# dusk-network/schnorr

Measured on NVIDIA B200. Metric: verifies_per_s, higher is better.
Workload: dtype u32

## Files before the change

### schnorr_b200/csrc/hades.cuh

```cuda
#pragma once
#include "fq.cuh"

namespace sb200 {

#define SB_HADES_W 5

struct HadesTables {
  uint32_t rc[335][8];
  uint32_t mds[25][8];
  uint32_t pre[5][8];
  uint32_t sparse[59 * 11][8];
  uint32_t post[25][8];
};
#if defined(__CUDACC__)
__constant__ HadesTables d_hades;
#endif
static HadesTables h_hades;

#if defined(__CUDA_ARCH__)
#define SB_CONST(name) d_##name
#define SB_HADES(field) d_hades.field
#else
#define SB_CONST(name) h_##name
#define SB_HADES(field) h_hades.field
#endif

SB_HD fq ld8(const uint32_t* p) {
  fq r;
#pragma unroll
  for (int i = 0; i < 8; i++) r.v[i] = p[i];
  return r;
}

SB_HD fq fq_pow5(const fq& x) {
  fq x2 = fq_sqr(x);
  fq x4 = fq_sqr(x2);
  return fq_mul(x4, x);
}

#define SB_MATMUL5(s, mat)                                                                  \
  do {                                                                                      \
    fq _r[5];                                                                               \
    _Pragma("unroll") for (int _k = 0; _k < 5; _k++)                                        \
        _r[_k] = fq_dot5(&SB_HADES(mat)[_k * 5], s[0], s[1], s[2], s[3], s[4]);             \
    _Pragma("unroll") for (int _k = 0; _k < 5; _k++) s[_k] = _r[_k];                        \
  } while (0)

#define SB_MATMUL5_PLAIN(s, mat)                                        \
  do {                                                                  \
    fq _r[5];                                                           \
    _Pragma("unroll 1") for (int _k = 0; _k < 5; _k++) {                \
      fq _a = fq_mul(ld8(SB_HADES(mat)[_k * 5]), s[0]);                 \
      _Pragma("unroll") for (int _j = 1; _j < 5; _j++)                  \
          _a = fq_add(_a, fq_mul(ld8(SB_HADES(mat)[_k * 5 + _j]), s[_j])); \
      _r[_k] = _a;                                                      \
    }                                                                   \
    _Pragma("unroll") for (int _k = 0; _k < 5; _k++) s[_k] = _r[_k];    \
  } while (0)

template <bool LAZY = true>
SB_HD void hades_full_round(fq* s, int rc_base) {
#pragma unroll
  for (int k = 0; k < 5; k++) s[k] = fq_pow5(fq_add(s[k], ld8(SB_HADES(rc)[rc_base + k])));
  if (LAZY) SB_MATMUL5(s, mds); else SB_MATMUL5_PLAIN(s, mds);
}

SB_HD void hades_perm_dense(fq* s) {
  int rc = 0;
#pragma unroll 1
  for (int r = 0; r < 4; r++, rc += 5) hades_full_round<false>(s, rc);
#pragma unroll 1
  for (int r = 0; r < 59; r++, rc += 5) {
#pragma unroll
    for (int k = 0; k < 5; k++) s[k] = fq_add(s[k], ld8(SB_HADES(rc)[rc + k]));
    s[4] = fq_pow5(s[4]);
    SB_MATMUL5_PLAIN(s, mds);
  }
#pragma unroll 1
  for (int r = 0; r < 4; r++, rc += 5) hades_full_round<false>(s, rc);
}

SB_HD void hades_perm(fq* s) {
  int rc = 0;
#pragma unroll 1
  for (int r = 0; r < 4; r++, rc += 5) hades_full_round(s, rc);
#pragma unroll
  for (int k = 0; k < 4; k++) s[k] = fq_add(s[k], ld8(SB_HADES(pre)[k]));
#pragma unroll 1
  for (int t = 0; t < 59; t++) {
    const uint32_t(*c)[8] = &SB_HADES(sparse)[t * 11];
    s[4] = fq_pow5(fq_add(s[4], ld8(c[0])));
    fq np = fq_dot5(&c[1], s[0], s[1], s[2], s[3], s[4]);
#pragma unroll
    for (int j = 0; j < 4; j++) s[j] = fq_add(s[j], fq_mul(ld8(c[6 + j]), s[4]));
    s[4] = np;
  }
  SB_MATMUL5(s, post);
  rc += 59 * 5;
#pragma unroll 1
  for (int r = 0; r < 4; r++, rc += 5) hades_full_round(s, rc);
}

SB_HD void truncate250(const fq& mont_word, uint32_t* c) {
  fq x = fq_from_mont(mont_word);
#pragma unroll
  for (int i = 0; i < 8; i++) c[i] = x.v[i];
  c[7] &= 0x03ffffffu;
}

template <bool DENSE = false>
SB_HD void challenge3(const fq& Ru, const fq& Rv, const fq& m, uint32_t* c) {
  fq s[5] = {fq_zero(), Ru, Rv, m, fq_one()};
  if (DENSE) hades_perm_dense(s); else hades_perm(s);
  truncate250(s[1], c);
}

template <bool DENSE = false>
SB_HD void challenge5(const fq& Ru, const fq& Rv, const fq& Rpu, const fq& Rpv, const fq& m, uint32_t* c) {
  fq s[5] = {fq_zero(), Ru, Rv, Rpu, Rpv};
  if (DENSE) hades_perm_dense(s); else hades_perm(s);
  s[1] = fq_add(s[1], m);
  s[2] = fq_add(s[2], fq_one());
  if (DENSE) hades_perm_dense(s); else hades_perm(s);
  truncate250(s[1], c);
}

}
```

### schnorr_b200/csrc/params_host.cuh

```cuda
#pragma once
#include <cstring>

#include "wire.cuh"

namespace sb200 {
namespace params {

struct Sha512 {
  static uint64_t rotr(uint64_t x, int n) { return (x >> n) | (x << (64 - n)); }
  static void digest(const uint8_t* msg, size_t len, uint8_t out[64]) {
    static const uint64_t K[80] = {
        0x428a2f98d728ae22ull, 0x7137449123ef65cdull, 0xb5c0fbcfec4d3b2full, 0xe9b5dba58189dbbcull, 0x3956c25bf348b538ull,
        0x59f111f1b605d019ull, 0x923f82a4af194f9bull, 0xab1c5ed5da6d8118ull, 0xd807aa98a3030242ull, 0x12835b0145706fbeull,
        0x243185be4ee4b28cull, 0x550c7dc3d5ffb4e2ull, 0x72be5d74f27b896full, 0x80deb1fe3b1696b1ull, 0x9bdc06a725c71235ull,
        0xc19bf174cf692694ull, 0xe49b69c19ef14ad2ull, 0xefbe4786384f25e3ull, 0x0fc19dc68b8cd5b5ull, 0x240ca1cc77ac9c65ull,
        0x2de92c6f592b0275ull, 0x4a7484aa6ea6e483ull, 0x5cb0a9dcbd41fbd4ull, 0x76f988da831153b5ull, 0x983e5152ee66dfabull,
        0xa831c66d2db43210ull, 0xb00327c898fb213full, 0xbf597fc7beef0ee4ull, 0xc6e00bf33da88fc2ull, 0xd5a79147930aa725ull,
        0x06ca6351e003826full, 0x142929670a0e6e70ull, 0x27b70a8546d22ffcull, 0x2e1b21385c26c926ull, 0x4d2c6dfc5ac42aedull,
        0x53380d139d95b3dfull, 0x650a73548baf63deull, 0x766a0abb3c77b2a8ull, 0x81c2c92e47edaee6ull, 0x92722c851482353bull,
        0xa2bfe8a14cf10364ull, 0xa81a664bbc423001ull, 0xc24b8b70d0f89791ull, 0xc76c51a30654be30ull, 0xd192e819d6ef5218ull,
        0xd69906245565a910ull, 0xf40e35855771202aull, 0x106aa07032bbd1b8ull, 0x19a4c116b8d2d0c8ull, 0x1e376c085141ab53ull,
        0x2748774cdf8eeb99ull, 0x34b0bcb5e19b48a8ull, 0x391c0cb3c5c95a63ull, 0x4ed8aa4ae3418acbull, 0x5b9cca4f7763e373ull,
        0x682e6ff3d6b2b8a3ull, 0x748f82ee5defb2fcull, 0x78a5636f43172f60ull, 0x84c87814a1f0ab72ull, 0x8cc702081a6439ecull,
        0x90befffa23631e28ull, 0xa4506cebde82bde9ull, 0xbef9a3f7b2c67915ull, 0xc67178f2e372532bull, 0xca273eceea26619cull,
        0xd186b8c721c0c207ull, 0xeada7dd6cde0eb1eull, 0xf57d4f7fee6ed178ull, 0x06f067aa72176fbaull, 0x0a637dc5a2c898a6ull,
        0x113f9804bef90daeull, 0x1b710b35131c471bull, 0x28db77f523047d84ull, 0x32caab7b40c72493ull, 0x3c9ebe0a15c9bebcull,
        0x431d67c49c100d4cull, 0x4cc5d4becb3e42b6ull, 0x597f299cfc657e2aull, 0x5fcb6fab3ad6faecull, 0x6c44198c4a475817ull};
    uint64_t h[8] = {0x6a09e667f3bcc908ull, 0xbb67ae8584caa73bull, 0x3c6ef372fe94f82bull, 0xa54ff53a5f1d36f1ull,
                     0x510e527fade682d1ull, 0x9b05688c2b3e6c1full, 0x1f83d9abfb41bd6bull, 0x5be0cd19137e2179ull};
    uint8_t buf[256];
    size_t total = ((len + 17 + 127) / 128) * 128;
    if (total > sizeof(buf)) return;
    memset(buf, 0, total);
    memcpy(buf, msg, len);
    buf[len] = 0x80;
    uint64_t bits = (uint64_t)len * 8;
    for (int i = 0; i < 8; i++) buf[total - 1 - i] = (uint8_t)(bits >> (8 * i));
    for (size_t off = 0; off < total; off += 128) {
      uint64_t w[80];
      for (int i = 0; i < 16; i++) {
        uint64_t x = 0;
        for (int k = 0; k < 8; k++) x = (x << 8) | buf[off + 8 * i + k];
        w[i] = x;
      }
      for (int i = 16; i < 80; i++) {
        uint64_t s0 = rotr(w[i - 15], 1) ^ rotr(w[i - 15], 8) ^ (w[i - 15] >> 7);
        uint64_t s1 = rotr(w[i - 2], 19) ^ rotr(w[i - 2], 61) ^ (w[i - 2] >> 6);
        w[i] = w[i - 16] + s0 + w[i - 7] + s1;
      }
      uint64_t a = h[0], b = h[1], c = h[2], d = h[3], e = h[4], f = h[5], g = h[6], hh = h[7];
      for (int i = 0; i < 80; i++) {
        uint64_t S1 = rotr(e, 14) ^ rotr(e, 18) ^ rotr(e, 41), ch = (e & f) ^ (~e & g);
        uint64_t t1 = hh + S1 + ch + K[i] + w[i];
        uint64_t S0 = rotr(a, 28) ^ rotr(a, 34) ^ rotr(a, 39), mj = (a & b) ^ (a & c) ^ (b & c);
        uint64_t t2 = S0 + mj;
        hh = g; g = f; f = e; e = d + t1; d = c; c = b; b = a; a = t1 + t2;
      }
      h[0] += a; h[1] += b; h[2] += c; h[3] += d; h[4] += e; h[5] += f; h[6] += g; h[7] += hh;
    }
    for (int i = 0; i < 8; i++)
      for (int k = 0; k < 8; k++) out[8 * i + k] = (uint8_t)(h[i] >> (56 - 8 * k));
  }
};

inline fq ld(const uint32_t* p) { fq r; memcpy(r.v, p, 32); return r; }
inline void st(uint32_t* p, const fq& a) { memcpy(p, a.v, 32); }
inline fq fq_small(uint32_t x) {
  fq c = fq_zero();
  c.v[0] = x;
  return fq_to_mont(c);
}

inline void default_round_constants(int rule, uint32_t (*out)[8], int n) {
  uint8_t bytes[64];
  const char* seed = "poseidon-for-plonk";
  size_t len = strlen(seed);
  memcpy(bytes, seed, len);
  fq p = fq_one();
  for (int i = 0; i < n; i++) {
    uint8_t d[64];
    Sha512::digest(bytes, len, d);
    memcpy(bytes, d, 64);
    len = 64;
    uint32_t w[16];
    memcpy(w, d, 64);
    fq h = fq_from_wide(w);
    if (rule == SB200_ARK_CUMSUM) {
      h = fq_add(h, p);
      p = h;
    }
    st(out[i], h);
  }
}

inline void default_mds(uint32_t (*out)[5][8]) {
  for (int i = 0; i < 5; i++)
    for (int j = 0; j < 5; j++) st(out[i][j], fq_inv(fq_small((uint32_t)(i + j + 5))));
}

struct Mat4 {
  fq a[4][4];
};
inline Mat4 mat_ident() {
  Mat4 m;
  for (int i = 0; i < 4; i++)
    for (int j = 0; j < 4; j++) m.a[i][j] = i == j ? fq_one() : fq_zero();
  return m;
}
inline Mat4 mat_mul(const Mat4& x, const Mat4& y) {
  Mat4 r;
  for (int i = 0; i < 4; i++)
    for (int j = 0; j < 4; j++) {
      fq s = fq_zero();
      for (int k = 0; k < 4; k++) s = fq_add(s, fq_mul(x.a[i][k], y.a[k][j]));
      r.a[i][j] = s;
    }
  return r;
}
inline void mat_vec(const Mat4& m, const fq* v, fq* out) {
  for (int i = 0; i < 4; i++) {
    fq s = fq_zero();
    for (int k = 0; k < 4; k++) s = fq_add(s, fq_mul(m.a[i][k], v[k]));
    out[i] = s;
  }
}
inline bool mat_inv(const Mat4& m, Mat4& out) {
  fq w[4][8];
  for (int i = 0; i < 4; i++)
    for (int j = 0; j < 8; j++) w[i][j] = j < 4 ? m.a[i][j] : (j - 4 == i ? fq_one() : fq_zero());
  for (int c = 0; c < 4; c++) {
    int piv = -1;
    for (int r = c; r < 4 && piv < 0; r++)
      if (!fq_is_zero(w[r][c])) piv = r;
    if (piv < 0) return false;
    if (piv != c)
      for (int j = 0; j < 8; j++) { fq t = w[c][j]; w[c][j] = w[piv][j]; w[piv][j] = t; }
    fq iv = fq_inv(w[c][c]);
    for (int j = 0; j < 8; j++) w[c][j] = fq_mul(w[c][j], iv);
    for (int r = 0; r < 4; r++) {
      if (r == c || fq_is_zero(w[r][c])) continue;
      fq f = w[r][c];
      for (int j = 0; j < 8; j++) w[r][j] = fq_sub(w[r][j], fq_mul(f, w[c][j]));
    }
  }
  for (int i = 0; i < 4; i++)
    for (int j = 0; j < 4; j++) out.a[i][j] = w[i][4 + j];
  return true;
}

inline bool derive_hades_tables(const uint32_t (*rc)[8], const uint32_t (*mds)[5][8], HadesTables& T) {
  constexpr int W = 5, P = 4, NP = 59, NF = 4;
  memcpy(T.rc, rc, sizeof(T.rc));
  memcpy(T.mds, mds, sizeof(T.mds));
  Mat4 Moo;
  fq Mop[4], Mpo[4], Mpp = ld(mds[P][P]);
  for (int i = 0; i < 4; i++) {
    for (int j = 0; j < 4; j++) Moo.a[i][j] = ld(mds[i][j]);
    Mop[i] = ld(mds[i][P]);
    Mpo[i] = ld(mds[P][i]);
  }
  static thread_local fq folds[NP][4], rows[NP][4], cols[NP][4], F[NP + 1][4];
  Mat4 B = mat_ident();
  for (int t = 0; t < NP; t++) {
    const uint32_t(*c)[8] = rc + (NF + t) * W;
    Mat4 Binv, Bn, Bninv;
    if (!mat_inv(B, Binv)) return false;
    fq co[4];
    for (int i = 0; i < 4; i++) co[i] = ld(c[i]);
    mat_vec(Binv, co, folds[t]);
    Bn = mat_mul(Moo, B);
    if (!mat_inv(Bn, Bninv)) return false;
    mat_vec(Bninv, Mop, cols[t]);
    for (int j = 0; j < 4; j++) {
      fq s = fq_zero();
      for (int k = 0; k < 4; k++) s = fq_add(s, fq_mul(Mpo[k], B.a[k][j]));
      rows[t][j] = s;
    }
    B = Bn;
  }
  for (int k = 0; k < 4; k++) F[0][k] = fq_zero();
  for (int t = 0; t < NP; t++)
    for (int k = 0; k < 4; k++) F[t + 1][k] = fq_add(F[t][k], folds[t][k]);
  for (int k = 0; k < 4; k++) st(T.pre[k], F[NP][k]);
  st(T.pre[P], fq_zero());
  for (int t = 0; t < NP; t++) {
    fq kP = ld(rc[(NF + t) * W + P]);
    if (t > 0) {
      fq corr = fq_zero();
      for (int k = 0; k < 4; k++) corr = fq_add(corr, fq_mul(rows[t - 1][k], fq_sub(F[NP][k], F[t][k])));
      kP = fq_sub(kP, corr);
    }
    uint32_t(*o)[8] = &T.sparse[t * 11];
    st(o[0], kP);
    for (int j = 0; j < 4; j++) st(o[1 + j], rows[t][j]);
    st(o[1 + P], Mpp);
    for (int j = 0; j < 4; j++) st(o[6 + j], cols[t][j]);
    st(o[6 + P], fq_zero());
  }
  for (int i = 0; i < W; i++)
    for (int j = 0; j < W; j++) {
      fq v = (i < 4 && j < 4) ? B.a[i][j] : (i == P && j == P ? fq_one() : fq_zero());
      st(T.post[i * W + j], v);
    }
  return true;
}

inline bool on_curve(const fq& u, const fq& v) {
  fq u2 = fq_sqr(u), v2 = fq_sqr(v);
  return fq_eq(fq_sub(v2, u2), fq_add(fq_one(), fq_mul(ed_d(), fq_mul(u2, v2))));
}
inline bool prime_order(const fq& u, const fq& v) {
  const uint32_t rr[8] = SB200_FR_MOD_INIT;
  ext base = affine_to_ext(u, v), acc = ext_identity();
  pniels nb = ext_to_pniels(base);
  for (int bit = 251; bit >= 0; bit--) {
    acc = p1p1_to_ext(ed_dbl(acc.X, acc.Y, acc.Z));
    if ((rr[bit >> 5] >> (bit & 31)) & 1u) acc = p1p1_to_ext(ed_add(acc, nb));
  }
  const bool is_id = fq_is_zero(acc.X) && fq_eq(acc.Y, acc.Z);
  const bool base_id = fq_is_zero(u) && fq_eq(v, fq_one());
  return is_id && !base_id;
}
inline bool canonical_fq(const uint32_t* p) { return lt_q(p); }

}
}
```

### schnorr_b200/csrc/schnorr_b200.cu

```cuda
#include <cuda_runtime.h>

#include <algorithm>
#include <atomic>
#include <cstdio>
#include <cstring>
#include <mutex>
#include <string>
#include <vector>

#include <map>
#include <thread>

#include "../../include/schnorr_b200.h"
#include "wire.cuh"
#include "params_host.cuh"

using namespace sb200;

namespace {

#ifndef SB_EC_GLOBAL_TABLES
#define SB_EC_GLOBAL_TABLES 1
#endif
constexpr int TPB = 128;
// ... 1075 lines not shown
    };
    for (int k = 0; k < d.nout; k++)
      if (d.out[k]) a.out[k] = dout[k] = (uint32_t*)carve(p, out_bytes(k));
    if (scr) {
      a.scratch = carve(p, scr);
      if (splits_with_scratch(d)) a.out[0] = (uint32_t*)a.scratch;
    }
    uint32_t* dbm = nullptr;
    if (d.bitmap) a.bitmap = dbm = (uint32_t*)carve(p, bm_bytes);
    if ((rc = launch(ctx, d.op, a, st))) return rc;
    auto d2h = [&](uint32_t* host_dst, const uint32_t* dev_src, size_t bytes, bool pinned) -> int {
      uint8_t* dst = (uint8_t*)host_dst;
      if (!pinned) {
        uint8_t* sp = carve(ho_p, bytes);
        dc.pending[slot].push_back({dst, sp, bytes});
        dst = sp;
      }
      CU(cudaMemcpyAsync(dst, dev_src, bytes, cudaMemcpyDeviceToHost, st));
      return SB200_OK;
    };
    for (int k = 0; k < d.nout; k++)
      if (d.out[k] && (rc = d2h(d.out_words[k] < 0 ? d.out[k] + c0 / 32 : d.out[k] + (size_t)c0 * d.out_words[k], dout[k],
                                out_bytes(k), d.out_words[k] < 0 ? bm_pinned : out_pinned[k])))
        return rc;
    if (d.bitmap && (rc = d2h(d.bitmap + c0 / 32, dbm, bm_bytes, bm_pinned))) return rc;
    CU(cudaEventRecord(dc.done[slot], st));
  }
  for (int s = 0; s < 2; s++) {
    int rc = drain_slot(ctx, dc, s);
    if (rc) return rc;
    CU(cudaStreamSynchronize(dc.stream[s]));
  }
  return SB200_OK;
}

void quiesce(DevCtx& dc) {
  cudaSetDevice(dc.dev);
  for (int s = 0; s < 2; s++) {
    if (dc.stream[s]) cudaStreamSynchronize(dc.stream[s]);
    dc.pending[s].clear();
  }
  cudaGetLastError();
}

int run(sb200_ctx* ctx, int64_t n, const Desc& d) {
  if (!ctx || n < 0) return SB200_ERR_ARG;
  uint32_t allowed = SB200_POINTS_AFFINE | SB200_DEVICE_PTRS;
  if (d.op == OP_VERIFY && SB_VERIFY_WS) allowed |= SB200_VERIFY_DUAL_PIPE;
  if (d.op == OP_VERIFY || d.op == OP_VERIFY_DOUBLE || d.op == OP_VERIFY_VARGEN) allowed |= SB200_CHECK_POINTS;
  if (d.op == OP_SIGN || d.op == OP_SIGN_DOUBLE || d.op == OP_SIGN_VARGEN || d.op == OP_KEYGEN || d.op == OP_KEYGEN_DOUBLE ||
      d.op == OP_KEYGEN_VARGEN)
    allowed |= SB200_SIGN_OBLIVIOUS;
  if (d.flags & ~allowed) return SB200_ERR_ARG;
  for (int k = 0; k < d.nin; k++)
    if (d.in_words[k] && (!d.in[k] || ((uintptr_t)d.in[k] & 15))) return SB200_ERR_ARG;
  for (int k = 0; k < d.nout; k++)
    if (d.out[k] && ((uintptr_t)d.out[k] & 15)) return SB200_ERR_ARG;
  if (n == 0) return SB200_OK;
  std::lock_guard<std::mutex> lock(ctx->mu);
  ctx->set_err("");
  DeviceGuard guard;

  if (d.flags & SB200_DEVICE_PTRS) {
    if (ctx->devs.size() != 1) return SB200_ERR_ARG;
    DevCtx& dc = ctx->devs[0];
    CU(cudaSetDevice(dc.dev));
    cudaStream_t st = ctx->user_stream;
    if (dc.user_ev_valid && dc.last_user_stream != st) CU(cudaStreamWaitEvent(st, dc.user_ev, 0));
    KArgs a{};
    a.n = n; a.flags = d.flags; a.aux = d.aux; a.combG = dc.combG; a.combGp = dc.combGp; a.bitmap = d.bitmap;
    a.comb4G = dc.comb4; a.comb4Gp = dc.comb4 + CT_TABLE_WORDS;
    a.ws = dc.ws[2]; a.nsm = dc.nsm; a.ec_scratch = dc.ec_scratch[2]; a.persist = ctx->persist;
    for (int k = 0; k < d.nin; k++) a.in[k] = d.in[k];
    for (int k = 0; k < d.nout; k++) a.out[k] = d.out[k];
    if (const size_t need = scratch_bytes(d, n)) {
      if (dc.cscratch_cap < need) {
        if (dc.user_ev_valid) CU(cudaEventSynchronize(dc.user_ev));
        if (dc.cscratch) CU(cudaFree(dc.cscratch));
        dc.cscratch = nullptr; dc.cscratch_cap = 0;
        if (cudaMalloc(&dc.cscratch, need) != cudaSuccess) { ctx->set_err("cudaMalloc scratch"); return SB200_ERR_NOMEM; }
        dc.cscratch_cap = need;
      }
      a.scratch = (uint8_t*)dc.cscratch;
      if (splits_with_scratch(d)) a.out[0] = dc.cscratch;
    }
    int rc = launch(ctx, d.op, a, st);
    if (rc) return rc;
    CU(cudaEventRecord(dc.user_ev, st));
    dc.user_ev_valid = true;
    dc.last_user_stream = st;
    return SB200_OK;
  }

  size_t per_tuple = 0;
  bool in_pinned[MAX_IN] = {}, out_pinned[MAX_OUT] = {}, bm_pinned = true;
  for (int k = 0; k < d.nin; k++) {
    per_tuple += (size_t)d.in_words[k] * 4;
    if (d.in_words[k]) in_pinned[k] = host_pinned(d.in[k]);
  }
  for (int k = 0; k < d.nout; k++) {
    per_tuple += (d.out[k] && d.out_words[k] > 0) ? (size_t)d.out_words[k] * 4 : 0;
    if (d.out[k]) out_pinned[k] = host_pinned(d.out[k]);
    if (d.out[k] && d.out_words[k] < 0) bm_pinned = bm_pinned && out_pinned[k];
  }
  if (d.bitmap) bm_pinned = bm_pinned && host_pinned(d.bitmap);

  const int ndev = (int)ctx->devs.size();
  const int64_t per_dev = ((n + ndev - 1) / ndev + 31) & ~(int64_t)31;
  std::vector<int> rcs(ndev, SB200_OK);
  auto work = [&](int di) {
    const int64_t lo = std::min<int64_t>(n, di * per_dev), hi = std::min<int64_t>(n, lo + per_dev);
    if (lo < hi) rcs[di] = run_device(ctx, ctx->devs[di], d, lo, hi, per_tuple, in_pinned, out_pinned, bm_pinned);
  };
  if (ndev == 1) {
    work(0);
  } else {
    std::vector<std::thread> th;
    for (int di = 1; di < ndev; di++) th.emplace_back(work, di);
    work(0);
    for (auto& t : th) t.join();
  }
  int rc = SB200_OK;
  for (int di = 0; di < ndev; di++)
    if (rcs[di] && !rc) rc = rcs[di];
  if (rc)
    for (auto& dc : ctx->devs) quiesce(dc);
  return rc;
}

int pt_words(uint32_t flags) { return (flags & SB200_POINTS_AFFINE) ? 16 : 24; }

void release_device(DevCtx& dc) {
  cudaSetDevice(dc.dev);
  for (int s = 0; s < 2; s++) {
    if (dc.stream[s]) { cudaStreamSynchronize(dc.stream[s]); cudaStreamDestroy(dc.stream[s]); }
    if (dc.done[s]) cudaEventDestroy(dc.done[s]);
    if (dc.arena[s]) cudaFree(dc.arena[s]);
    if (dc.hin[s].p) cudaFreeHost(dc.hin[s].p);
    if (dc.hout[s].p) cudaFreeHost(dc.hout[s].p);
  }
  if (dc.user_ev) { if (dc.user_ev_valid) cudaEventSynchronize(dc.user_ev); cudaEventDestroy(dc.user_ev); }
  if (dc.combG) cudaFree(dc.combG);
  if (dc.combGp) cudaFree(dc.combGp);
  if (dc.comb4) cudaFree(dc.comb4);
  for (int s = 0; s < 3; s++) {
    if (dc.ws[s]) cudaFree(dc.ws[s]);
    if (dc.ec_scratch[s]) cudaFree(dc.ec_scratch[s]);
  }
  if (dc.cscratch) cudaFree(dc.cscratch);
  if (dc.registered) {
    std::lock_guard<std::mutex> l(g_params_mu);
    auto it = g_dev_params.find(dc.dev);
    if (it != g_dev_params.end() && --it->second.refs <= 0) g_dev_params.erase(it);
  }
  dc = DevCtx();
}

int prepare_params(const sb200_params* p, HadesTables& T) {
  if (!p || p->struct_size != sizeof(sb200_params) || p->reserved != 0) return SB200_ERR_ARG;
  const uint32_t* all = p->generator;
  const size_t nfe = (sizeof(sb200_params) - 8) / 32;
  for (size_t i = 0; i < nfe; i++)
    if (!params::canonical_fq(all + 8 * i)) return SB200_ERR_PARAMS;
  const fq gu = params::ld(p->generator), gv = params::ld(p->generator + 8);
  const fq hu = params::ld(p->generator_nums), hv = params::ld(p->generator_nums + 8);
  if (!params::on_curve(gu, gv) || !params::on_curve(hu, hv)) return SB200_ERR_PARAMS;
  if (!params::prime_order(gu, gv) || !params::prime_order(hu, hv)) return SB200_ERR_PARAMS;
  if (!params::derive_hades_tables(p->round_constants, p->mds, T)) return SB200_ERR_PARAMS;
  h_hades = T;
  uint64_t s = 0x9e3779b97f4a7c15ull;
  for (int trial = 0; trial < 3; trial++) {
    fq a[5], b[5];
    for (int k = 0; k < 5; k++) {
      for (int j = 0; j < 8; j++) { s ^= s << 13; s ^= s >> 7; s ^= s << 17; a[k].v[j] = trial ? (uint32_t)s : 0u; }
      a[k].v[7] &= 0x3fffffffu;
      b[k] = a[k];
    }
    hades_perm_dense(a);
    hades_perm(b);
    for (int k = 0; k < 5; k++)
      if (!fq_eq(a[k], b[k])) return SB200_ERR_PARAMS;
  }
  return SB200_OK;
}

}

extern "C" {

int sb200_default_params(int ark_rule, sb200_params* out) {
  if (!out) return SB200_ERR_ARG;
  if (ark_rule == SB200_ARK_ENV) {
    const char* e = getenv("SB200_ARK");
    ark_rule = (e && !strcmp(e, "plain")) ? SB200_ARK_PLAIN : SB200_ARK_CUMSUM;
    if (e && strcmp(e, "plain") && strcmp(e, "cumsum") && *e) return SB200_ERR_ARG;
  }
  if (ark_rule != SB200_ARK_CUMSUM && ark_rule != SB200_ARK_PLAIN) return SB200_ERR_ARG;
  memset(out, 0, sizeof(*out));
  out->struct_size = sizeof(sb200_params);
  const uint32_t g[4][8] = {SB200_G_U_INIT, SB200_G_V_INIT, SB200_GP_U_INIT, SB200_GP_V_INIT};
  memcpy(out->generator, g[0], 32); memcpy(out->generator + 8, g[1], 32);
  memcpy(out->generator_nums, g[2], 32); memcpy(out->generator_nums + 8, g[3], 32);
  params::default_round_constants(ark_rule, out->round_constants, 335);
  params::default_mds(out->mds);
  return SB200_OK;
}

int sb200_init(const int* devices, int n_devices, sb200_ctx** out) {
  sb200_params p;
  int rc = sb200_default_params(SB200_ARK_ENV, &p);
  if (rc) return rc;
  return sb200_init_ex(&p, devices, n_devices, out);
}

int sb200_init_ex(const sb200_params* params_in, const int* devices, int n_devices, sb200_ctx** out) {
  if (!out || n_devices < 0 || (n_devices > 0 && !devices)) return SB200_ERR_ARG;
  *out = nullptr;
  sb200_ctx* ctx = new sb200_ctx();
  auto fail = [&](int code) { sb200_destroy(ctx); return code; };
  int rc = prepare_params(params_in, ctx->tables);
  if (rc) return fail(rc);
  ctx->params = *params_in;
  if (const char* e = getenv("SB200_CURVE_PERSISTENT")) ctx->persist = !strcmp(e, "always") ? 1 : !strcmp(e, "never") ? 2 : 0;
  int count = 0;
  if (cudaGetDeviceCount(&count) != cudaSuccess || count == 0) return fail(SB200_ERR_NODEV);
  DeviceGuard guard;
  int dflt = 0;
  if (n_devices == 0) { devices = &dflt; n_devices = 1; }
  const uint64_t hash = fnv1a(params_in, sizeof(*params_in));
  const fq gu = params::ld(params_in->generator), gv = params::ld(params_in->generator + 8);
  const fq hu = params::ld(params_in->generator_nums), hv = params::ld(params_in->generator_nums + 8);
  ctx->devs.reserve(n_devices);
  for (int i = 0; i < n_devices; i++) {
    if (devices[i] < 0 || devices[i] >= count) return fail(SB200_ERR_ARG);
    cudaDeviceProp prop;
    if (cudaGetDeviceProperties(&prop, devices[i]) != cudaSuccess || prop.major < 10) return fail(SB200_ERR_NODEV);
    ctx->devs.emplace_back();
    DevCtx& dc = ctx->devs.back();
    dc.dev = devices[i];
    if (cudaSetDevice(dc.dev) != cudaSuccess) return fail(SB200_ERR_CUDA);
    {
      std::lock_guard<std::mutex> l(g_params_mu);
      DevParams& dp = g_dev_params[dc.dev];
      if (dp.refs > 0 && dp.hash != hash) return fail(SB200_ERR_BUSY);
      if (dp.refs == 0 || dp.hash != hash) {
        if (cudaMemcpyToSymbol(d_hades, &ctx->tables, sizeof(HadesTables)) != cudaSuccess) return fail(SB200_ERR_CUDA);
        dp.hash = hash;
      }
      dp.refs++;
      dc.registered = true;
    }
    for (int s = 0; s < 2; s++) {
      if (cudaStreamCreateWithFlags(&dc.stream[s], cudaStreamNonBlocking) != cudaSuccess) return fail(SB200_ERR_CUDA);
      if (cudaEventCreateWithFlags(&dc.done[s], cudaEventDisableTiming) != cudaSuccess) return fail(SB200_ERR_CUDA);
    }
    if (cudaEventCreateWithFlags(&dc.user_ev, cudaEventDisableTiming) != cudaSuccess) return fail(SB200_ERR_CUDA);
    size_t tb = (size_t)COMB_WINDOWS * COMB_ENTRIES * 24 * 4;
    if (cudaMalloc(&dc.combG, tb) != cudaSuccess || cudaMalloc(&dc.combGp, tb) != cudaSuccess) return fail(SB200_ERR_NOMEM);
    if (cudaMalloc(&dc.comb4, (size_t)2 * CT_TABLE_WORDS * 4) != cudaSuccess) return fail(SB200_ERR_NOMEM);
    if (cudaFuncSetAttribute(k_fixed_batch<OP_SIGN_DOUBLE, true>, cudaFuncAttributeMaxDynamicSharedMemorySize, 2 * CT_TABLE_WORDS * 4) != cudaSuccess ||
        cudaFuncSetAttribute(k_fixed_batch<OP_KEYGEN_DOUBLE, true>, cudaFuncAttributeMaxDynamicSharedMemorySize, 2 * CT_TABLE_WORDS * 4) != cudaSuccess ||
        cudaFuncSetAttribute(k_fixed_batch<OP_SIGN, true>, cudaFuncAttributeMaxDynamicSharedMemorySize, CT_TABLE_WORDS * 4) != cudaSuccess ||
        cudaFuncSetAttribute(k_fixed_batch<OP_KEYGEN, true>, cudaFuncAttributeMaxDynamicSharedMemorySize, CT_TABLE_WORDS * 4) != cudaSuccess)
      return fail(SB200_ERR_CUDA);
    dc.nsm = prop.multiProcessorCount;
#if SB_VERIFY_WS
    if (cudaFuncSetAttribute(k_verify_ws, cudaFuncAttributeMaxDynamicSharedMemorySize, (int)WS_SMEM) != cudaSuccess) return fail(SB200_ERR_CUDA);
#endif
#if SB_VERIFY_WS || SB_EC_GLOBAL_TABLES
    for (int s = 0; s < 3; s++)
      if (cudaMalloc(&dc.ws[s], sizeof(WsState)) != cudaSuccess || cudaMemset(dc.ws[s], 0, sizeof(WsState)) != cudaSuccess)
        return fail(SB200_ERR_NOMEM);
#endif
#if SB_EC_GLOBAL_TABLES
    for (int s = 0; s < 3; s++)
      if (cudaMalloc(&dc.ec_scratch[s], (size_t)(SB_EC_P_CTAS0 > 4 ? SB_EC_P_CTAS0 : 4) * dc.nsm * TPB * EC_P_ENTRIES * sizeof(pniels)) != cudaSuccess) return fail(SB200_ERR_NOMEM);
    if (cudaFuncSetAttribute(k_curve_p<2>, cudaFuncAttributeMaxDynamicSharedMemorySize, (int)ec_p_smem(2)) != cudaSuccess) return fail(SB200_ERR_CUDA);
#endif
    int grid = (COMB_WINDOWS * COMB_ENTRIES + TPB - 1) / TPB;
    k_comb_build<<<grid, TPB, 0, dc.stream[0]>>>(dc.combG, gu, gv);
    k_comb_build<<<grid, TPB, 0, dc.stream[0]>>>(dc.combGp, hu, hv);
    k_comb4_build<<<(CT_WINDOWS * CT_ENTRIES + TPB - 1) / TPB, TPB, 0, dc.stream[0]>>>(dc.comb4, gu, gv);
    k_comb4_build<<<(CT_WINDOWS * CT_ENTRIES + TPB - 1) / TPB, TPB, 0, dc.stream[0]>>>(dc.comb4 + CT_TABLE_WORDS, hu, hv);
    ctx->launches += 4;
  }
  for (auto& dc : ctx->devs)
    if (cudaSetDevice(dc.dev) != cudaSuccess || cudaStreamSynchronize(dc.stream[0]) != cudaSuccess) return fail(SB200_ERR_CUDA);
  *out = ctx;
  return SB200_OK;
}

void sb200_destroy(sb200_ctx* ctx) {
  if (!ctx) return;
  {
    DeviceGuard guard;
    for (auto& dc : ctx->devs) release_device(dc);
  }
  delete ctx;
}

int sb200_params_check(const sb200_params* params_in, uint32_t* tables_out) {
  HadesTables* T = new HadesTables();
  int rc = prepare_params(params_in, *T);
  if (!rc && tables_out) memcpy(tables_out, T, sizeof(HadesTables));
  delete T;
  return rc;
}
int sb200_get_params(const sb200_ctx* ctx, sb200_params* out) {
  if (!ctx || !out) return SB200_ERR_ARG;
  *out = ctx->params;
  return SB200_OK;
}
int sb200_dbg_hades_tables(const sb200_ctx* ctx, uint32_t* out) {
  if (!ctx || !out) return SB200_ERR_ARG;
  memcpy(out, &ctx->tables, sizeof(HadesTables));
  return SB200_OK;
}

const char* sb200_strerror(int code) {
  switch (code) {
    case SB200_OK: return "ok";
    case SB200_ERR_ARG: return "invalid argument";
    case SB200_ERR_CUDA: return "CUDA error";
    case SB200_ERR_NODEV: return "no usable sm_100 CUDA device";
    case SB200_ERR_NOMEM: return "out of device memory";
    case SB200_ERR_PARAMS: return "scheme parameters rejected";
    case SB200_ERR_BUSY: return "device already holds different scheme parameters";
    default: return "unknown error";
  }
}
const char* sb200_last_error(const sb200_ctx* ctx) { return ctx ? ctx->err.c_str() : ""; }
int sb200_device_count(const sb200_ctx* ctx) { return ctx ? (int)ctx->devs.size() : 0; }
int sb200_set_stream(sb200_ctx* ctx, void* s) {
  if (!ctx) return SB200_ERR_ARG;
  ctx->user_stream = (cudaStream_t)s;
  return SB200_OK;
}
uint64_t sb200_launch_count(const sb200_ctx* ctx) { return ctx ? ctx->launches.load() : 0; }
int sb200_host_alloc(size_t bytes, void** out) {
  if (!out) return SB200_ERR_ARG;
  return cudaHostAlloc(out, bytes, cudaHostAllocPortable) == cudaSuccess ? SB200_OK : SB200_ERR_NOMEM;
}
void sb200_host_free(void* p) { if (p) cudaFreeHost(p); }

#define IN(k, ptr, words) d.in[k] = (ptr); d.in_words[k] = (words)
#define OUT(k, ptr, words) d.out[k] = (ptr); d.out_words[k] = (words)

int sb200_verify(sb200_ctx* ctx, int64_t n, uint32_t flags, const uint32_t* pk, const uint32_t* sig_u, const uint32_t* sig_R,
                 const uint32_t* msg, uint32_t* verdicts, uint32_t* c_out) {
  if (!verdicts) return SB200_ERR_ARG;
  Desc d; d.op = OP_VERIFY; d.flags = flags; d.nin = 4; d.nout = 1; d.bitmap = verdicts;
  IN(0, pk, pt_words(flags)); IN(1, sig_u, 8); IN(2, sig_R, pt_words(flags)); IN(3, msg, 8); OUT(0, c_out, 8);
  return run(ctx, n, d);
}
int sb200_verify_double(sb200_ctx* ctx, int64_t n, uint32_t flags, const uint32_t* pk, const uint32_t* pkp, const uint32_t* sig_u,
                        const uint32_t* sig_R, const uint32_t* sig_Rp, const uint32_t* msg, uint32_t* verdicts, uint32_t* c_out) {
  if (!verdicts) return SB200_ERR_ARG;
  Desc d; d.op = OP_VERIFY_DOUBLE; d.flags = flags; d.nin = 6; d.nout = 1; d.bitmap = verdicts;
  int pw = pt_words(flags);
  IN(0, pk, pw); IN(1, pkp, pw); IN(2, sig_u, 8); IN(3, sig_R, pw); IN(4, sig_Rp, pw); IN(5, msg, 8); OUT(0, c_out, 8);
  return run(ctx, n, d);
}
int sb200_verify_vargen(sb200_ctx* ctx, int64_t n, uint32_t flags, const uint32_t* pk, const uint32_t* gen, const uint32_t* sig_u,
                        const uint32_t* sig_R, const uint32_t* msg, uint32_t* verdicts, uint32_t* c_out) {
  if (!verdicts) return SB200_ERR_ARG;
  Desc d; d.op = OP_VERIFY_VARGEN; d.flags = flags; d.nin = 5; d.nout = 1; d.bitmap = verdicts;
  int pw = pt_words(flags);
  IN(0, pk, pw); IN(1, gen, pw); IN(2, sig_u, 8); IN(3, sig_R, pw); IN(4, msg, 8); OUT(0, c_out, 8);
  return run(ctx, n, d);
}
int sb200_sign(sb200_ctx* ctx, int64_t n, uint32_t flags, const uint32_t* sk, const uint32_t* msg, const uint32_t* nonce,
               uint32_t* u_out, uint32_t* R_out, uint32_t* c_out) {
  if (!u_out || !R_out) return SB200_ERR_ARG;
  Desc d; d.op = OP_SIGN; d.flags = flags; d.nin = 3; d.nout = 4;
  IN(0, sk, 8); IN(1, msg, 8); IN(2, nonce, 8); OUT(0, u_out, 8); OUT(1, R_out, 16); OUT(3, c_out, 8);
  return run(ctx, n, d);
}
int sb200_sign_double(sb200_ctx* ctx, int64_t n, uint32_t flags, const uint32_t* sk, const uint32_t* msg, const uint32_t* nonce,
                      uint32_t* u_out, uint32_t* R_out, uint32_t* Rp_out, uint32_t* c_out) {
  if (!u_out || !R_out || !Rp_out) return SB200_ERR_ARG;
  Desc d; d.op = OP_SIGN_DOUBLE; d.flags = flags; d.nin = 3; d.nout = 4;
  IN(0, sk, 8); IN(1, msg, 8); IN(2, nonce, 8); OUT(0, u_out, 8); OUT(1, R_out, 16); OUT(2, Rp_out, 16); OUT(3, c_out, 8);
  return run(ctx, n, d);
}
int sb200_sign_vargen(sb200_ctx* ctx, int64_t n, uint32_t flags, const uint32_t* sk, const uint32_t* gen, const uint32_t* msg,
                      const uint32_t* nonce, uint32_t* u_out, uint32_t* R_out, uint32_t* c_out) {
  if (!u_out || !R_out) return SB200_ERR_ARG;
  Desc d; d.op = OP_SIGN_VARGEN; d.flags = flags; d.nin = 4; d.nout = 4;
  IN(0, sk, 8); IN(1, gen, pt_words(flags)); IN(2, msg, 8); IN(3, nonce, 8); OUT(0, u_out, 8); OUT(1, R_out, 16); OUT(3, c_out, 8);
  return run(ctx, n, d);
}
int sb200_keygen(sb200_ctx* ctx, int64_t n, uint32_t flags, const uint32_t* sk, uint32_t* pk_out) {
  if (!pk_out) return SB200_ERR_ARG;
  Desc d; d.op = OP_KEYGEN; d.flags = flags; d.nin = 1; d.nout = 1;
  IN(0, sk, 8); OUT(0, pk_out, 16);
  return run(ctx, n, d);
}
int sb200_keygen_double(sb200_ctx* ctx, int64_t n, uint32_t flags, const uint32_t* sk, uint32_t* pk_out, uint32_t* pkp_out) {
  if (!pk_out || !pkp_out) return SB200_ERR_ARG;
  Desc d; d.op = OP_KEYGEN_DOUBLE; d.flags = flags; d.nin = 1; d.nout = 2;
  IN(0, sk, 8); OUT(0, pk_out, 16); OUT(1, pkp_out, 16);
  return run(ctx, n, d);
}
int sb200_keygen_vargen(sb200_ctx* ctx, int64_t n, uint32_t flags, const uint32_t* sk, const uint32_t* gen, uint32_t* pk_out) {
  if (!pk_out) return SB200_ERR_ARG;
  Desc d; d.op = OP_KEYGEN_VARGEN; d.flags = flags; d.nin = 2; d.nout = 1;
  IN(0, sk, 8); IN(1, gen, pt_words(flags)); OUT(0, pk_out, 16);
  return run(ctx, n, d);
}
int sb200_points_decompress(sb200_ctx* ctx, int64_t n, uint32_t flags, const uint8_t* bytes, uint32_t* points_out, uint32_t* ok_bitmap) {
  if (!points_out || !ok_bitmap || (flags & SB200_POINTS_AFFINE)) return SB200_ERR_ARG;
  Desc d; d.op = OP_DECOMPRESS; d.flags = flags; d.nin = 1; d.nout = 1; d.bitmap = ok_bitmap;
  IN(0, (const uint32_t*)bytes, 8); OUT(0, points_out, 16);
  return run(ctx, n, d);
}
int sb200_points_compress(sb200_ctx* ctx, int64_t n, uint32_t flags, const uint32_t* points, uint8_t* bytes_out) {
  if (!bytes_out) return SB200_ERR_ARG;
  Desc d; d.op = OP_COMPRESS; d.flags = flags; d.nin = 1; d.nout = 1;
  IN(0, points, pt_words(flags)); OUT(0, (uint32_t*)bytes_out, 8);
  return run(ctx, n, d);
}
int sb200_scalars_from_wide(sb200_ctx* ctx, int64_t n, uint32_t flags, int field, const uint8_t* wide, uint32_t* out) {
  if (!out || field < 0 || field > 1 || (flags & SB200_POINTS_AFFINE)) return SB200_ERR_ARG;
  Desc d; d.op = OP_FROM_WIDE; d.flags = flags; d.aux = field; d.nin = 1; d.nout = 1;
  IN(0, (const uint32_t*)wide, 16); OUT(0, out, 8);
  return run(ctx, n, d);
}
int sb200_fq_to_mont(sb200_ctx* ctx, int64_t n, uint32_t flags, const uint32_t* in, uint32_t* out) {
  if (!out || (flags & SB200_POINTS_AFFINE)) return SB200_ERR_ARG;
  Desc d; d.op = OP_DBG_FQ; d.flags = flags; d.aux = 5; d.nin = 2; d.nout = 1;
  IN(0, in, 8); IN(1, nullptr, 0); OUT(0, out, 8);
  return run(ctx, n, d);
}
int sb200_fq_from_mont(sb200_ctx* ctx, int64_t n, uint32_t flags, const uint32_t* in, uint32_t* out) {
  if (!out || (flags & SB200_POINTS_AFFINE)) return SB200_ERR_ARG;
  Desc d; d.op = OP_DBG_FQ; d.flags = flags; d.aux = 6; d.nin = 2; d.nout = 1;
  IN(0, in, 8); IN(1, nullptr, 0); OUT(0, out, 8);
  return run(ctx, n, d);
}
int sb200_verify_bytes(sb200_ctx* ctx, int64_t n, uint32_t flags, const uint8_t* pk, const uint8_t* sig, const uint8_t* msg,
                       uint32_t* verdicts, uint32_t* invalid) {
  if (!verdicts || (flags & SB200_POINTS_AFFINE)) return SB200_ERR_ARG;
  Desc d; d.op = OP_VERIFY_BYTES; d.flags = flags | SB200_POINTS_AFFINE; d.nin = 3; d.nout = 1; d.bitmap = verdicts;
  IN(0, (const uint32_t*)pk, 8); IN(1, (const uint32_t*)sig, 16); IN(2, (const uint32_t*)msg, 8);
  d.out[0] = invalid; d.out_words[0] = -1;
  return run(ctx, n, d);
}
int sb200_sign_bytes(sb200_ctx* ctx, int64_t n, uint32_t flags, const uint8_t* sk, const uint8_t* msg, const uint8_t* nonce,
                     uint8_t* sig_out, uint32_t* invalid) {
  if (!sig_out || (flags & SB200_POINTS_AFFINE)) return SB200_ERR_ARG;
  Desc d; d.op = OP_SIGN_BYTES; d.flags = flags; d.nin = 3; d.nout = 1; d.bitmap = invalid;
  IN(0, (const uint32_t*)sk, 8); IN(1, (const uint32_t*)msg, 8); IN(2, (const uint32_t*)nonce, 8); OUT(0, (uint32_t*)sig_out, 16);
  return run(ctx, n, d);
}
int sb200_verify_double_bytes(sb200_ctx* ctx, int64_t n, uint32_t flags, const uint8_t* pk, const uint8_t* sig, const uint8_t* msg,
                              uint32_t* verdicts, uint32_t* invalid) {
  if (!verdicts || (flags & SB200_POINTS_AFFINE)) return SB200_ERR_ARG;
  Desc d; d.op = OP_VERIFY_DOUBLE_BYTES; d.flags = flags | SB200_POINTS_AFFINE; d.nin = 3; d.nout = 1; d.bitmap = verdicts;
  IN(0, (const uint32_t*)pk, 16); IN(1, (const uint32_t*)sig, 24); IN(2, (const uint32_t*)msg, 8);
  d.out[0] = invalid; d.out_words[0] = -1;
  return run(ctx, n, d);
}
int sb200_verify_vargen_bytes(sb200_ctx* ctx, int64_t n, uint32_t flags, const uint8_t* pk, const uint8_t* sig, const uint8_t* msg,
                              uint32_t* verdicts, uint32_t* invalid) {
  if (!verdicts || (flags & SB200_POINTS_AFFINE)) return SB200_ERR_ARG;
  Desc d; d.op = OP_VERIFY_VARGEN_BYTES; d.flags = flags | SB200_POINTS_AFFINE; d.nin = 3; d.nout = 1; d.bitmap = verdicts;
  IN(0, (const uint32_t*)pk, 16); IN(1, (const uint32_t*)sig, 16); IN(2, (const uint32_t*)msg, 8);
  d.out[0] = invalid; d.out_words[0] = -1;
  return run(ctx, n, d);
}
int sb200_sign_double_bytes(sb200_ctx* ctx, int64_t n, uint32_t flags, const uint8_t* sk, const uint8_t* msg, const uint8_t* nonce,
                            uint8_t* sig_out, uint32_t* invalid) {
  if (!sig_out || (flags & SB200_POINTS_AFFINE)) return SB200_ERR_ARG;
  Desc d; d.op = OP_SIGN_DOUBLE_BYTES; d.flags = flags; d.nin = 3; d.nout = 1; d.bitmap = invalid;
  IN(0, (const uint32_t*)sk, 8); IN(1, (const uint32_t*)msg, 8); IN(2, (const uint32_t*)nonce, 8); OUT(0, (uint32_t*)sig_out, 24);
  return run(ctx, n, d);
}
int sb200_sign_vargen_bytes(sb200_ctx* ctx, int64_t n, uint32_t flags, const uint8_t* sk, const uint8_t* msg, const uint8_t* nonce,
                            uint8_t* sig_out, uint32_t* invalid) {
  if (!sig_out || (flags & SB200_POINTS_AFFINE)) return SB200_ERR_ARG;
  Desc d; d.op = OP_SIGN_VARGEN_BYTES; d.flags = flags | SB200_POINTS_AFFINE; d.nin = 3; d.nout = 1; d.bitmap = invalid;
  IN(0, (const uint32_t*)sk, 16); IN(1, (const uint32_t*)msg, 8); IN(2, (const uint32_t*)nonce, 8); OUT(0, (uint32_t*)sig_out, 16);
  return run(ctx, n, d);
}
int sb200_sign_witness(sb200_ctx* ctx, int64_t n, uint32_t flags, int scheme, const uint32_t* sk, const uint32_t* msg,
                       const uint32_t* nonce, const uint32_t* generator, uint32_t* rows_out) {
  if (!rows_out || scheme < 0 || scheme > 2 || (scheme == 2 && !generator)) return SB200_ERR_ARG;
  if (scheme != 2 && (flags & SB200_POINTS_AFFINE)) return SB200_ERR_ARG;
  static const int width[3] = {11, 19, 13};
  Desc d; d.op = OP_WITNESS; d.flags = flags; d.aux = scheme; d.nin = 4; d.nout = 1;
  IN(0, sk, 8); IN(1, msg, 8); IN(2, nonce, 8); IN(3, scheme == 2 ? generator : nullptr, scheme == 2 ? pt_words(flags) : 0);
  OUT(0, rows_out, 8 * width[scheme]);
  return run(ctx, n, d);
}
int sb200_points_check(sb200_ctx* ctx, int64_t n, uint32_t flags, const uint32_t* points, uint32_t* ok_bitmap) {
  if (!ok_bitmap) return SB200_ERR_ARG;
  Desc d; d.op = OP_POINTS_CHECK; d.flags = flags; d.nin = 1; d.nout = 0; d.bitmap = ok_bitmap;
  IN(0, points, pt_words(flags));
  return run(ctx, n, d);
}
int sb200_dbg_verify_ec(sb200_ctx* ctx, int64_t n, uint32_t flags, const uint32_t* pk, const uint32_t* sig_u, const uint32_t* sig_R,
                        const uint32_t* c, uint32_t* verdicts) {
  if (!verdicts) return SB200_ERR_ARG;
  Desc d; d.op = OP_DBG_VERIFY_EC; d.flags = flags; d.nin = 4; d.nout = 0; d.bitmap = verdicts;
  IN(0, pk, pt_words(flags)); IN(1, sig_u, 8); IN(2, sig_R, pt_words(flags)); IN(3, c, 8);
  return run(ctx, n, d);
}
int sb200_dbg_fq(sb200_ctx* ctx, int64_t n, int op, const uint32_t* a, const uint32_t* b, uint32_t* out) {
  if (!out || op < 0 || op > 7) return SB200_ERR_ARG;
  Desc d; d.op = OP_DBG_FQ; d.flags = 0; d.aux = op; d.nin = 2; d.nout = 1;
  IN(0, a, 8); IN(1, b, b ? 8 : 0); OUT(0, out, 8);
  return run(ctx, n, d);
}
int sb200_dbg_lattice3(sb200_ctx* ctx, int64_t n, const uint32_t* c, const uint32_t* u, uint32_t* out) {
  if (!out) return SB200_ERR_ARG;
  Desc d; d.op = OP_DBG_LAT3; d.flags = 0; d.nin = 2; d.nout = 1;
  IN(0, c, 8); IN(1, u, 8); OUT(0, out, 32);
  return run(ctx, n, d);
}
int sb200_dbg_fr_mul(sb200_ctx* ctx, int64_t n, const uint32_t* a, const uint32_t* b, uint32_t* out) {
  if (!out) return SB200_ERR_ARG;
  Desc d; d.op = OP_DBG_FR_MUL; d.flags = 0; d.nin = 2; d.nout = 1;
  IN(0, a, 8); IN(1, b, 8); OUT(0, out, 8);
  return run(ctx, n, d);
}
int sb200_dbg_hades(sb200_ctx* ctx, int64_t n, int dense, uint32_t* states) {
  if (!states || dense < 0 || dense > (SB_EXPERIMENTAL_FD ? 2 : 1)) return SB200_ERR_ARG;
  Desc d; d.op = OP_DBG_HADES; d.flags = 0; d.aux = dense; d.nin = 1; d.nout = 1;
  IN(0, states, 40); OUT(0, states, 40);
  return run(ctx, n, d);
}
int sb200_dbg_scalar_mul(sb200_ctx* ctx, int64_t n, uint32_t flags, int base, const uint32_t* points, const uint32_t* k, uint32_t* out) {
  if (!out || base < 0 || base > 2 || (base == 2 && !points)) return SB200_ERR_ARG;
  Desc d; d.op = OP_DBG_SMUL; d.flags = flags; d.aux = base; d.nin = 2; d.nout = 1;
  IN(0, points, base == 2 ? pt_words(flags) : 0); IN(1, k, 8); OUT(0, out, 16);
  return run(ctx, n, d);
}

}
```

Baseline: 24.88 million.

## Compute Hades linear layers as scaled small-integer matrix via FP64 FMA limbs

When every entry of the inverse MDS matrix is a small integer, the host builds a scaled integer matrix L/d together with rescaled round constants, per-round fix-up factors and a final unscale factor. On the device, each of the 67 rounds then applies the linear layer with FP64 FMAs on 32-bit limbs, followed by a cheap quotient-estimate reduction. This replaces the Montgomery multiplications in the matrix step with floating-point integer arithmetic. The cost is a full 5x5 layer and an extra multiply in every partial round, in place of the sparse partial-round form, and correctness depends on the limb bounds holding exactly.

Result: faster. 28.80 million (median of 6 runs) (+15.8%).

```diff
diff --git a/schnorr_b200/csrc/hades.cuh b/schnorr_b200/csrc/hades.cuh
--- a/schnorr_b200/csrc/hades.cuh
+++ b/schnorr_b200/csrc/hades.cuh
@@ -1,4 +1,9 @@
 #pragma once
+#include <cstddef>
+#include <cstring>
+#if !defined(__CUDA_ARCH__)
+#include <cmath>
+#endif
 #include "fq.cuh"
 
 namespace sb200 {
@@ -11,7 +16,14 @@
   uint32_t pre[5][8];
   uint32_t sparse[59 * 11][8];
   uint32_t post[25][8];
+  double cmat[25];
+  uint32_t src[335][8];
+  uint32_t fix[59][8];
+  uint32_t unscale[8];
+  uint32_t int_layers;
 };
+constexpr size_t HADES_ABI_BYTES = 1039 * 32;
+static_assert(offsetof(HadesTables, cmat) == HADES_ABI_BYTES, "the public table views keep their offsets");
 #if defined(__CUDACC__)
 __constant__ HadesTables d_hades;
 #endif
@@ -80,7 +92,115 @@
   for (int r = 0; r < 4; r++, rc += 5) hades_full_round<false>(s, rc);
 }
 
+constexpr uint32_t HI_2P52 = 0x43300000u;
+constexpr double RECIP_Q224 = 0x1.1aa84a76ff6f1p-31;
+
+SB_HD double hl_fma(double a, double b, double c) {
+#if defined(__CUDA_ARCH__)
+  return __fma_rn(a, b, c);
+#else
+  SB_COUNT(dfma, 1);
+  return std::fma(a, b, c);
+#endif
+}
+SB_HD double hl_pair(uint32_t hi, uint32_t lo) {
+#if defined(__CUDA_ARCH__)
+  return __hiloint2double((int)hi, (int)lo);
+#else
+  uint64_t b = (uint64_t)hi << 32 | lo;
+  double d;
+  memcpy(&d, &b, 8);
+  return d;
+#endif
+}
+SB_HD uint64_t hl_bits(double d) {
+#if defined(__CUDA_ARCH__)
+  return (uint64_t)__double_as_longlong(d);
+#else
+  uint64_t b;
+  memcpy(&b, &d, 8);
+  return b;
+#endif
+}
+SB_HD double hl_sub52(double d) {
+#if defined(__CUDA_ARCH__)
+  return __dsub_rn(d, 0x1p+52);
+#else
+  return d - 0x1p+52;
+#endif
+}
+
+SB_HD void hl_reduce(fq& r, uint32_t top) {
+  const double T = hl_sub52(hl_pair(HI_2P52 | top, r.v[7]));
+#if defined(__CUDA_ARCH__)
+  const double h = __fma_rz(T, RECIP_Q224, 0x1p+52);
+#else
+  SB_COUNT(dfma, 1);
+  const uint64_t Ti = (uint64_t)top << 32 | r.v[7];
+  const double h = 0x1p+52 + (double)(uint64_t)(((unsigned __int128)Ti * 0x11aa84a76ff6f1ull) >> 83);
+#endif
+  const double Qd = hl_sub52(h);
+  uint32_t lo[8], hi[8];
+  lo[0] = (uint32_t)hl_bits(h);
+  hi[0] = 0;
+#pragma unroll
+  for (int i = 1; i < 8; i++) {
+    const uint64_t b = hl_bits(hl_fma(Qd, (double)FqP::p(i), 0x1p+52));
+    lo[i] = (uint32_t)b;
+    hi[i] = (uint32_t)(b >> 32) & 0xfffffu;
+  }
+  uint32_t qq[8], sh[8];
+  sh[0] = 0;
+#pragma unroll
+  for (int i = 1; i < 8; i++) sh[i] = hi[i - 1];
+  add8(qq, lo, sh);
+  sub8(r.v, r.v, qq);
+  cond_sub_p<FqP>(r.v);
+}
+
+SB_HD void hades_int_layer(fq* s) {
+  uint32_t c[5];
+#pragma unroll
+  for (int i = 0; i < 8; i++) {
+    double x[5];
+#pragma unroll
+    for (int j = 0; j < 5; j++) x[j] = hl_sub52(hl_pair(HI_2P52, s[j].v[i]));
+#pragma unroll
+    for (int k = 0; k < 5; k++) {
+      double acc = hl_pair(HI_2P52, i ? c[k] : 0u);
+#pragma unroll
+      for (int j = 0; j < 5; j++) acc = hl_fma(SB_HADES(cmat)[k * 5 + j], x[j], acc);
+      const uint64_t b = hl_bits(acc);
+      s[k].v[i] = (uint32_t)b;
+      c[k] = (uint32_t)(b >> 32) & 0xfffffu;
+    }
+  }
+#pragma unroll
+  for (int k = 0; k < 5; k++) hl_reduce(s[k], c[k]);
+}
+
+SB_HD void hades_perm_int(fq* s) {
+#pragma unroll 1
+  for (int r = 0; r < 67; r++) {
+#pragma unroll
+    for (int k = 0; k < 5; k++) s[k] = fq_add(s[k], ld8(SB_HADES(src)[r * 5 + k]));
+    if (r < 4 || r >= 63) {
+#pragma unroll
+      for (int k = 0; k < 5; k++) s[k] = fq_pow5(s[k]);
+    } else {
+      s[4] = fq_mul(fq_pow5(s[4]), ld8(SB_HADES(fix)[r - 4]));
+    }
+    hades_int_layer(s);
+  }
+#pragma unroll
+  for (int k = 0; k < 5; k++) s[k] = fq_mul(s[k], ld8(SB_HADES(unscale)));
+}
+
 SB_HD void hades_perm(fq* s) {
+  if (SB_HADES(int_layers)) {
+    hades_perm_int(s);
+    return;
+  }
   int rc = 0;
 #pragma unroll 1
   for (int r = 0; r < 4; r++, rc += 5) hades_full_round(s, rc);
diff --git a/schnorr_b200/csrc/params_host.cuh b/schnorr_b200/csrc/params_host.cuh
--- a/schnorr_b200/csrc/params_host.cuh
+++ b/schnorr_b200/csrc/params_host.cuh
@@ -148,6 +148,45 @@
   return true;
 }
 
+constexpr uint32_t INT_LAYER_CMAX_BOUND = (1u << 20) / 5;
+
+inline void derive_int_tables(HadesTables& T) {
+  constexpr int W = 5, NP = 59, NF = 4;
+  memset(T.cmat, 0, sizeof(T.cmat));
+  memset(T.src, 0, sizeof(T.src));
+  memset(T.fix, 0, sizeof(T.fix));
+  memset(T.unscale, 0, sizeof(T.unscale));
+  T.int_layers = 0;
+  uint64_t d[25], L = 1, cmax = 0;
+  for (int e = 0; e < 25; e++) {
+    const fq iv = fq_from_mont(fq_inv(ld(T.mds[e])));
+    for (int i = 1; i < 8; i++)
+      if (iv.v[i]) return;
+    if (iv.v[0] == 0 || iv.v[0] >= INT_LAYER_CMAX_BOUND) return;
+    d[e] = iv.v[0];
+    uint64_t a = L, b = d[e];
+    while (b) { uint64_t t = a % b; a = b; b = t; }
+    L = L / a * d[e];
+    if (L >= (1ull << 32)) return;
+  }
+  for (int e = 0; e < 25; e++) cmax = L / d[e] > cmax ? L / d[e] : cmax;
+  if (cmax >= INT_LAYER_CMAX_BOUND) return;
+  for (int e = 0; e < 25; e++) T.cmat[e] = (double)(L / d[e]);
+  const fq Lf = fq_small((uint32_t)L);
+  fq tau = fq_one();
+  for (int r = 0; r < 2 * NF + NP; r++) {
+    for (int k = 0; k < W; k++) st(T.src[r * W + k], fq_mul(ld(T.rc[r * W + k]), tau));
+    if (r < NF || r >= NF + NP) {
+      tau = fq_mul(fq_sqr(fq_sqr(tau)), tau);
+    } else {
+      st(T.fix[r - NF], fq_inv(fq_sqr(fq_sqr(tau))));
+    }
+    tau = fq_mul(tau, Lf);
+  }
+  st(T.unscale, fq_inv(tau));
+  T.int_layers = 1;
+}
+
 inline bool derive_hades_tables(const uint32_t (*rc)[8], const uint32_t (*mds)[5][8], HadesTables& T) {
   constexpr int W = 5, P = 4, NP = 59, NF = 4;
   memcpy(T.rc, rc, sizeof(T.rc));
@@ -202,6 +241,7 @@
       fq v = (i < 4 && j < 4) ? B.a[i][j] : (i == P && j == P ? fq_one() : fq_zero());
       st(T.post[i * W + j], v);
     }
+  derive_int_tables(T);
   return true;
 }
 
diff --git a/schnorr_b200/csrc/schnorr_b200.cu b/schnorr_b200/csrc/schnorr_b200.cu
--- a/schnorr_b200/csrc/schnorr_b200.cu
+++ b/schnorr_b200/csrc/schnorr_b200.cu
@@ -1401,7 +1401,7 @@
 int sb200_params_check(const sb200_params* params_in, uint32_t* tables_out) {
   HadesTables* T = new HadesTables();
   int rc = prepare_params(params_in, *T);
-  if (!rc && tables_out) memcpy(tables_out, T, sizeof(HadesTables));
+  if (!rc && tables_out) memcpy(tables_out, T, HADES_ABI_BYTES);
   delete T;
   return rc;
 }
@@ -1412,7 +1412,7 @@
 }
 int sb200_dbg_hades_tables(const sb200_ctx* ctx, uint32_t* out) {
   if (!ctx || !out) return SB200_ERR_ARG;
-  memcpy(out, &ctx->tables, sizeof(HadesTables));
+  memcpy(out, &ctx->tables, HADES_ABI_BYTES);
   return SB200_OK;
 }
 
```
